# Kinetica-jl/Kinetica.jl

Measured on AMD Instinct MI355X. Metric: RHS evals/sec (batched sweep) + wall-clock per solve_network, 10k-species CRN, higher is better.
Workload: dtype f64; 1 GPU; synthetic CRN 10000 species / 50000 reactions (seed 12345), batched RHS sweep, B=4096 states per GPU with per-state Arrhenius k (500-1200 K); states_per_gpu=4096, parallelism=replicas x1 (no data-path collective)

## Files before the change

### kinetica_jl_amd/csrc/tiled_api.cpp

```cpp
#include "../../include/kinetica_hip.h"

#include <algorithm>
#include <cstdio>
#include <cmath>

#include "handle.hpp"
#include "tiled_kernels.hpp"

using namespace kin;

namespace {

int tiled_block_size(int64_t N) {
  return N <= 2300 ? 256 : (N <= 4850 ? 512 : 1024);
}

void ensure_tiled(kin_network* h) {
  if (!h->tiled_tried) {
    h->tiled_tried = true;
    h->tiled = build_tiled(h->host, tiled_block_size(h->host.N), 0);
    const TiledHost& L = h->tiled;
    if (L.ok) {
      hipStream_t s = h->stream;
      std::vector<int32_t> rxn_of_slot((size_t)L.k_len(), -1);
      for (int32_t r = 0; r < L.R; r++) if (L.slot_of_reaction[r] >= 0) rxn_of_slot[L.slot_of_reaction[r]] = r;
      h->t_rec.upload(L.rec, s);
      h->t_copy.upload(L.copy_src, s);
      h->t_kf.upload(L.kf, s); h->t_kr.upload(L.kr, s); h->t_rxn_of_slot.upload(rxn_of_slot, s); h->t_kslot.upload(L.kslot, s);
      h->t_spec_of_lib.upload(L.species_of_lib, s); h->t_lib_of_spec.upload(L.lib_of_species, s);
      if (!L.identity) { h->t_stage_lib.upload(L.stage_lib, s); h->t_stage_off.upload(L.stage_off, s); }
      KIN_HIP(hipStreamSynchronize(s));
    }
  }
  if (!h->tiled.ok) throw KinError(ERR_UNSUPPORTED, "network has no tiled layout: " + h->tiled.why);
}

void ensure_params(kin_network* h, hipStream_t) {
  if (!h->has_arrhenius) throw KinError(ERR_STATE, "Arrhenius parameters were never set");
  if (h->t_par_valid) return;
  const TiledHost& L = h->tiled;
  KIN_HIP(hipDeviceSynchronize());
  h->t_par.alloc((size_t)4 * std::max(1, L.P));
  launch_tiled_params(L.P, h->t_kf.p, h->t_kr.p, h->Ea.p, h->A.p, h->has_kmax, h->t_mult, h->t_par.p, h->stream);
  KIN_HIP(hipStreamSynchronize(h->stream));
  h->t_par_valid = true;
}

TiledView view_of(kin_network* h) {
  const TiledHost& L = h->tiled;
  TiledView v{};
  v.KL = L.KL; v.has_singles = L.has_singles ? 1 : 0;
  v.N = L.N; v.P = L.P; v.h = L.h; v.n_copy = L.n_copy; v.wbase = L.wbase; v.E = L.E; v.T = L.T;
  v.win_cnt_max = 0;
  for (int32_t c : L.win_cnt) v.win_cnt_max = std::max(v.win_cnt_max, c);
  v.rec = (const uint2*)h->t_rec.p;
  for (int32_t t = 0; t < L.T; t++) {
    v.seginfo[t] = make_int4(L.seginfo[4 * t], L.seginfo[4 * t + 1], L.seginfo[4 * t + 2], L.seginfo[4 * t + 3]);
    v.segk[t] = L.seg_k[2 * t];
    v.win_off[t] = L.win_off[t]; v.win_cnt[t] = L.win_cnt[t];
  }
  v.copy_src = h->t_copy.p;
  v.par = (const double4*)h->t_par.p;
  v.has_kmax = h->has_kmax ? 1 : 0;
  v.inv_kmax = h->has_kmax ? 1.0 / h->k_max : 0.0;
  return v;
}

void require(bool c, int code, const char* msg) {
  if (!c) throw KinError(code, msg);
}

void states_convert(kin_network* h, int64_t B, bool to_lib, const double* d_in, double* d_out, hipStream_t s) {
  const int64_t N = h->host.N;
  if (h->tiled.identity) KIN_HIP(hipMemcpyAsync(d_out, d_in, (size_t)B * N * sizeof(double), hipMemcpyDeviceToDevice, s));
  else launch_permute_staged(N, B, to_lib, h->t_stage_lib.p, h->t_stage_off.p, d_in, d_out, s);
}

}

#define KIN_TRY(h) try { KIN_HIP(hipSetDevice((h)->device));
#define KIN_CATCH(h)                                                        \
  }                                                                         \
  catch (const KinError& e) { (h)->err = e.what(); return e.code; }         \
  catch (const std::exception& e) { (h)->err = e.what(); return KIN_ERR_DEVICE; } \
  return KIN_OK;

extern "C" {

int kin_lib_layout(kin_network* h, int index_base, int64_t* k_len, int64_t* species_of_lib, int64_t* slot_of_reaction,
                   int32_t* species_identity, int64_t* info) {
  if (!h) return KIN_ERR_INVALID_ARG;
  KIN_TRY(h)
  ensure_tiled(h);
  const TiledHost& L = h->tiled;
  if (k_len) *k_len = L.k_len();
  if (species_of_lib) for (int32_t j = 0; j < L.N; j++) species_of_lib[j] = L.species_of_lib[j] + index_base;
  if (slot_of_reaction) for (int32_t r = 0; r < L.R; r++) slot_of_reaction[r] = L.slot_of_reaction[r] + index_base;
  if (species_identity) *species_identity = L.identity ? 1 : 0;
  if (info) { info[0] = L.h; info[1] = L.T; info[2] = L.P; info[3] = L.E; info[4] = L.n_copy; info[5] = L.BS; }
  KIN_CATCH(h)
}

int kin_lib_layout_host(int64_t n_species, int64_t n_reactions, const int64_t* reac_ptr, const int64_t* reac_idx,
                        const int64_t* reac_sto, const int64_t* prod_ptr, const int64_t* prod_idx, const int64_t* prod_sto,
                        int index_base, int hubs, int64_t* info, int64_t* species_of_lib, int64_t* slot_of_reaction,
                        uint64_t* rec, int32_t* rowtab, int32_t* seg_q, int32_t* win_off, int32_t* win_cnt, int32_t* copy_src,
                        int32_t* seg_k) {
  try {
    const NetworkHost H = compile_network(n_species, n_reactions, reac_ptr, reac_idx, reac_sto, prod_ptr, prod_idx, prod_sto, index_base);
    const TiledHost L = build_tiled(H, tiled_block_size(H.N), hubs);
    if (!L.ok) {
      if (getenv("KIN_TILED_DEBUG")) fprintf(stderr, "[tiled] no layout: %s\n", L.why.c_str());
      return KIN_ERR_UNSUPPORTED;
    }
    if (info) {
      info[0] = L.h; info[1] = L.T; info[2] = L.P; info[3] = L.E; info[4] = L.n_copy; info[5] = L.BS; info[6] = L.wbase;
      info[7] = L.seg_q.back(); info[8] = L.k_len(); info[9] = L.has_singles ? 1 : 0;
    }
    if (species_of_lib) for (int32_t j = 0; j < L.N; j++) species_of_lib[j] = L.species_of_lib[j];
    if (slot_of_reaction) for (int32_t r = 0; r < L.R; r++) slot_of_reaction[r] = L.slot_of_reaction[r];
    if (rec) for (int32_t p = 0; p < L.P; p++) rec[p] = (uint64_t)L.rec[2 * p] | ((uint64_t)L.rec[2 * p + 1] << 32);
    if (rowtab) std::copy(L.rowtab.begin(), L.rowtab.end(), rowtab);
    if (seg_q) std::copy(L.seg_q.begin(), L.seg_q.end(), seg_q);
    if (win_off) std::copy(L.win_off.begin(), L.win_off.end(), win_off);
    if (win_cnt) std::copy(L.win_cnt.begin(), L.win_cnt.end(), win_cnt);
    if (copy_src) std::copy(L.copy_src.begin(), L.copy_src.end(), copy_src);
    if (seg_k) std::copy(L.seg_k.begin(), L.seg_k.end(), seg_k);
  } catch (const KinError& e) {
    return e.code;
  } catch (const std::exception&) {
    return KIN_ERR_INVALID_ARG;
  }
  return KIN_OK;
}

int kin_states_to_lib_dev(kin_network* h, int64_t B, const double* d_in, double* d_out, void* stream) {
  if (!h) return KIN_ERR_INVALID_ARG;
  KIN_TRY(h)
  require(B > 0 && d_in && d_out && d_in != d_out, ERR_INVALID_ARG, "bad arguments");
  ensure_tiled(h);
  states_convert(h, B, true, d_in, d_out, stream ? (hipStream_t)stream : h->stream);
  KIN_CATCH(h)
}

int kin_states_from_lib_dev(kin_network* h, int64_t B, const double* d_in, double* d_out, void* stream) {
  if (!h) return KIN_ERR_INVALID_ARG;
  KIN_TRY(h)
  require(B > 0 && d_in && d_out && d_in != d_out, ERR_INVALID_ARG, "bad arguments");
  ensure_tiled(h);
  states_convert(h, B, false, d_in, d_out, stream ? (hipStream_t)stream : h->stream);
  KIN_CATCH(h)
}

int kin_rates_to_lib_dev(kin_network* h, int64_t B, const double* d_k, double* d_k_lib, void* stream) {
  if (!h) return KIN_ERR_INVALID_ARG;
  KIN_TRY(h)
  require(B > 0 && d_k && d_k_lib && d_k != d_k_lib, ERR_INVALID_ARG, "bad arguments");
  ensure_tiled(h);
  hipStream_t s = stream ? (hipStream_t)stream : h->stream;
  const TiledHost& L = h->tiled;
  if (L.KL == 2 * (int64_t)L.P && h->host.R % 2 == 0 && ((((uintptr_t)d_k) | ((uintptr_t)d_k_lib)) & 15) == 0)
    launch_rates_to_lib_pairs(L.P, h->host.R, B, h->t_kf.p, h->t_kr.p, d_k, d_k_lib, s);
  else
    launch_gather_rows(L.k_len(), h->host.R, B, h->t_rxn_of_slot.p, d_k, d_k_lib, s);
  KIN_CATCH(h)
}

int kin_rate_table_lib_dev(kin_network* h, const double* T, int64_t n_stops, double* d_out) {
  if (!h) return KIN_ERR_INVALID_ARG;
  KIN_TRY(h)
  require(T != nullptr && d_out != nullptr && n_stops >= 0, ERR_INVALID_ARG, "bad arguments");
  ensure_tiled(h);
  ensure_params(h, h->stream);
  h->T_stops.upload(T, n_stops, h->stream);
  TiledPadSlots pads{};
  for (int32_t q : h->tiled.pad_slots) pads.slot[pads.n++] = q;
  launch_rate_table_lib(h->tiled.P, h->tiled.KL, n_stops, h->t_par.p, h->t_kslot.p, pads, h->has_kmax, h->k_max, h->T_stops.p, d_out, h->stream);
  KIN_HIP(hipStreamSynchronize(h->stream));
  KIN_CATCH(h)
}

int kin_rhs_tiled_dev(kin_network* h, int64_t B, const double* d_u_lib, const double* d_k_lib, const double* d_T,
                      double* d_du_lib, void* stream) {
  if (!h) return KIN_ERR_INVALID_ARG;
  KIN_TRY(h)
  require(B > 0 && d_u_lib && d_du_lib, ERR_INVALID_ARG, "bad arguments");
  require((d_k_lib != nullptr) != (d_T != nullptr), ERR_INVALID_ARG, "exactly one of d_k_lib and d_T must be given");
  require((((uintptr_t)d_k_lib) & 15) == 0, ERR_INVALID_ARG, "d_k_lib must be 16-byte aligned");
  ensure_tiled(h);
  hipStream_t s = stream ? (hipStream_t)stream : h->stream;
  if (d_T) ensure_params(h, s);
  if (h->tiled.P == 0) {
    KIN_HIP(hipMemsetAsync(d_du_lib, 0, (size_t)B * h->host.N * sizeof(double), s));
    return KIN_OK;
  }
  launch_tiled_sweep(view_of(h), h->tiled.BS, h->n_cu, B, d_u_lib, d_k_lib, d_T, d_du_lib, s);
  KIN_CATCH(h)
}

int kin_rhs_batched_T_dev(kin_network* h, int64_t B, const double* d_u, const double* d_T, double* d_du, void* stream) {
  if (!h) return KIN_ERR_INVALID_ARG;
  KIN_TRY(h)
  require(B > 0 && d_u && d_T && d_du, ERR_INVALID_ARG, "bad arguments");
  ensure_tiled(h);
  hipStream_t s = stream ? (hipStream_t)stream : h->stream;
  ensure_params(h, s);
  const int64_t N = h->host.N;
  if (h->tiled.P == 0) {
    KIN_HIP(hipMemsetAsync(d_du, 0, (size_t)B * N * sizeof(double), s));
    return KIN_OK;
  }
  if (h->tiled.identity) {
    launch_tiled_sweep(view_of(h), h->tiled.BS, h->n_cu, B, d_u, nullptr, d_T, d_du, s);
  } else {
    h->t_u.alloc((size_t)B * N); h->t_du.alloc((size_t)B * N);
    states_convert(h, B, true, d_u, h->t_u.p, s);
    launch_tiled_sweep(view_of(h), h->tiled.BS, h->n_cu, B, h->t_u.p, nullptr, d_T, h->t_du.p, s);
    states_convert(h, B, false, h->t_du.p, d_du, s);
  }
  KIN_CATCH(h)
}

int kin_rhs_batched_klib_dev(kin_network* h, int64_t B, const double* d_u, const double* d_k_lib, double* d_du, void* stream) {
  if (!h) return KIN_ERR_INVALID_ARG;
  KIN_TRY(h)
  require(B > 0 && d_u && d_k_lib && d_du, ERR_INVALID_ARG, "bad arguments");
  require((((uintptr_t)d_k_lib) & 15) == 0, ERR_INVALID_ARG, "d_k_lib must be 16-byte aligned");
  ensure_tiled(h);
  hipStream_t s = stream ? (hipStream_t)stream : h->stream;
  const int64_t N = h->host.N;
  if (h->tiled.P == 0) {
    KIN_HIP(hipMemsetAsync(d_du, 0, (size_t)B * N * sizeof(double), s));
    return KIN_OK;
  }
  if (h->tiled.identity) {
    launch_tiled_sweep(view_of(h), h->tiled.BS, h->n_cu, B, d_u, d_k_lib, nullptr, d_du, s);
  } else {
    h->t_u.alloc((size_t)B * N); h->t_du.alloc((size_t)B * N);
    states_convert(h, B, true, d_u, h->t_u.p, s);
    launch_tiled_sweep(view_of(h), h->tiled.BS, h->n_cu, B, h->t_u.p, d_k_lib, nullptr, h->t_du.p, s);
    states_convert(h, B, false, h->t_du.p, d_du, s);
  }
  KIN_CATCH(h)
}

}
```

### kinetica_jl_amd/csrc/tiled_kernels.hip

```cpp
#include "tiled_kernels.hpp"

#include "exp_tab.hpp"

#ifndef KIN_TILED_SUB
#define KIN_TILED_SUB 2
#endif

namespace kin {

namespace {

template <bool TMODE, int NB_> struct Batch;
template <int NB_> struct Batch<false, NB_> { static constexpr int NB = NB_; double2 k[NB]; uint2 w[NB]; };
template <int NB_> struct Batch<true, NB_> { static constexpr int NB = NB_; double4 p[NB]; uint2 w[NB]; };

struct Labels { uint32_t l0, l1, l2, l3; };
__device__ __forceinline__ Labels decode(uint2 w) {
  return Labels{w.x & 0x3fffu, (w.x >> 14) & 0x3fffu, (w.x >> 28) | ((w.y & 0x3ffu) << 4), (w.y >> 10) & 0x3fffu};
}

}

template <int BS, bool TMODE, int UN, bool SINGLES>
__global__ __launch_bounds__(BS) void tiled_sweep_kernel(TiledView v, int B, const double* __restrict__ u,
                                                         const double* __restrict__ k_lib, const double* __restrict__ Tb,
                                                         double* __restrict__ du) {
  extern __shared__ double lds[];
  double* du_s = lds;
  double* u_s = lds + v.E;
  const double* tab_s = lds + 2 * v.E;
  const int tid = threadIdx.x;
  const int N = v.N, h = v.h, wbase = v.wbase, T = v.T;
  const size_t KL = (size_t)v.KL;

  for (int i = tid; i < v.E; i += BS) du_s[i] = 0.0;
  if (tid < TILED_DUMMY) u_s[h + tid] = 1.0;
  if (TMODE) for (int i = tid; i < TILED_EXP_TAB; i += BS) lds[2 * v.E + i] = kExp2Tab[i * (512 / TILED_EXP_TAB)];
  const int csrc = tid < v.n_copy ? v.copy_src[min(tid, max(v.n_copy - 1, 0))] : -1;
  const uint64_t dl = (uint64_t)(h + (tid & 63));
  const uint64_t ew = dl | (dl << 14) | (dl << 28) | (dl << 42) | (4ull << 56);
  const uint2 EMPTY = {(uint32_t)ew, (uint32_t)(ew >> 32)};

  const int Bm1 = B - 1;
  double un[UN];
  auto load_hubs = [&](int bb) {
    const double* ub = u + (size_t)min(bb, Bm1) * N;
#pragma unroll
    for (int x = 0; x < UN; x++) un[x] = ub[min(tid + x * BS, h - 1)];
  };
  auto store_hubs = [&]() {
#pragma unroll
    for (int x = 0; x < UN; x++) {
      const int e = tid + x * BS;
      if (e < h) u_s[e] = un[x];
    }
  };
  auto load_window = [&](int bb, int s) {
    const double* ub = u + (size_t)bb * N + v.win_off[s];
    const int cm1 = v.win_cnt[s] - 1;
#pragma unroll
    for (int x = 0; x < UN; x++) un[x] = ub[min(tid + x * BS, cm1)];
  };
  auto store_window = [&](int s) {
    const int c = v.win_cnt[s];
#pragma unroll
    for (int x = 0; x < UN; x++) {
      const int e = tid + x * BS;
      if (e < c) u_s[wbase + e] = un[x];
    }
  };

  constexpr int NB = (TMODE || UN > 5) ? 2 : 4;
  using BatchT = Batch<TMODE, NB>;
  static_assert(TILED_MIN_ROWS >= 2 * NB && (UN > 5 ? 2 : 4) % NB == 0, "segments are padded to whole batches, two at least");
  int pb = blockIdx.x, ps = 0, pi = 0;
  int4 pa = v.seginfo[0], pn = v.seginfo[T > 1 ? 1 : 0];
  int pak = SINGLES ? v.segk[0] : 0, pnk = SINGLES ? v.segk[T > 1 ? 1 : 0] : 0;
  asm volatile("" : "+s"(pa.x), "+s"(pa.y), "+s"(pa.z), "+s"(pn.x), "+s"(pn.y), "+s"(pn.z));
  if constexpr (SINGLES) asm volatile("" : "+s"(pa.w), "+s"(pn.w), "+s"(pak), "+s"(pnk));
  auto load_batch = [&](BatchT& G) {
    if (pi >= pa.z) {
      pi = 0; pa = pn; pak = pnk;
      if (++ps == T) { ps = 0; pb += gridDim.x; }
    }
    const bool live = pb < B;
    const double* kb = TMODE ? nullptr : k_lib + (size_t)min(pb, Bm1) * KL;
#pragma unroll
    for (int x = 0; x < NB; x++) {
      const int off = (pi + x) * BS + tid;
      const bool ok = live && off < pa.y;
      const int p = ok ? pa.x + off : 0;
      const uint2 w = v.rec[p];
      G.w[x].x = ok ? w.x : EMPTY.x;
      G.w[x].y = ok ? w.y : EMPTY.y;
      if constexpr (TMODE) G.p[x] = v.par[p];
      else if constexpr (!SINGLES) G.k[x] = *reinterpret_cast<const double2*>(kb + 2 * (size_t)p);
      else {
        const bool one = (off & ~63) >= pa.w;
        const size_t e = !ok ? 0 : (one ? (size_t)(pak + pa.w) + (size_t)(off & ~1) : (size_t)pak + 2 * (size_t)off);
        const double2 kk = *reinterpret_cast<const double2*>(kb + e);
        const bool odd = one && (off & 1);
        const int lo = odd ? __double2loint(kk.y) : __double2loint(kk.x), hi = odd ? __double2hiint(kk.y) : __double2hiint(kk.x);
        const int rlo = one ? 0 : __double2loint(kk.y), rhi = one ? 0 : __double2hiint(kk.y);
        G.k[x].x = __hiloint2double(hi, lo);
        G.k[x].y = __hiloint2double(rhi, rlo);
      }
    }
    pi += NB;
  };

  double RT = 1.0, inv_RT = 1.0;
#if defined(KIN_TILED_PROBE)
  double probe_acc = 0.0;
#endif
  auto consume = [&](const BatchT& G) {
    constexpr int SUB = KIN_TILED_SUB < NB ? KIN_TILED_SUB : NB;
#pragma unroll
    for (int x0 = 0; x0 < NB; x0 += SUB) {
      uint32_t fl[SUB];
      double net[SUB];
#pragma unroll
      for (int y = 0; y < SUB; y++) {
        const int x = x0 + y;
        fl[y] = __builtin_amdgcn_readfirstlane(G.w[x].y >> 24);
        const Labels L = decode(G.w[x]);
#if defined(KIN_TILED_SKIPREAD)
        double u1v = 1.0, u3v = 1.0;
        const double u0v = u_s[L.l0];
        if (fl[y] & 1u) u1v = u_s[L.l1];
        const double u2v = u_s[L.l2];
        if (fl[y] & 2u) u3v = u_s[L.l3];
        const double uf = u0v * u1v, ur = u2v * u3v;
#elif defined(KIN_TILED_PROBE) && (KIN_TILED_PROBE == 1 || KIN_TILED_PROBE == 3)
        const double uf = 1.0 + (double)L.l0, ur = 1.0 + (double)L.l2;
#else
        const double uf = u_s[L.l0] * u_s[L.l1];
        const double ur = u_s[L.l2] * u_s[L.l3];
#endif
        double kf, kr;
        if constexpr (TMODE) {
          kf = arrhenius_fast_t<TILED_EXP_TAB>(G.p[x].x, G.p[x].y, G.p[x].y, RT, inv_RT, v.has_kmax, v.inv_kmax, tab_s);
          kr = arrhenius_fast_t<TILED_EXP_TAB>(G.p[x].z, G.p[x].w, G.p[x].w, RT, inv_RT, v.has_kmax, v.inv_kmax, tab_s);
        } else {
          kf = G.k[x].x; kr = G.k[x].y;
        }
        net[y] = kf * uf - kr * ur;
      }
#pragma unroll
      for (int y = 0; y < SUB; y++) {
        if (fl[y] & 4u) continue;
        const Labels L = decode(G.w[x0 + y]);
#if defined(KIN_TILED_PROBE)
        probe_acc += net[y];
        continue;
#endif
        __hip_atomic_fetch_add(du_s + L.l0, -net[y], __ATOMIC_RELAXED, __HIP_MEMORY_SCOPE_WORKGROUP);
        if (fl[y] & 1u) __hip_atomic_fetch_add(du_s + L.l1, -net[y], __ATOMIC_RELAXED, __HIP_MEMORY_SCOPE_WORKGROUP);
        __hip_atomic_fetch_add(du_s + L.l2, net[y], __ATOMIC_RELAXED, __HIP_MEMORY_SCOPE_WORKGROUP);
        if (fl[y] & 2u) __hip_atomic_fetch_add(du_s + L.l3, net[y], __ATOMIC_RELAXED, __HIP_MEMORY_SCOPE_WORKGROUP);
      }
    }
  };

  int b = blockIdx.x;
  load_hubs(b);
  const int csrc_c = max(csrc, 0);
  double ucn = u[(size_t)min(b, Bm1) * N + csrc_c];
  double Tn = TMODE ? Tb[min(b, Bm1)] : 1.0;
  BatchT G0, G1;
  load_batch(G0);
  load_batch(G1);

  for (; b < B; b += gridDim.x) {
    double* dub = du + (size_t)b * N;
    const int bn = b + gridDim.x;
    if (TMODE) { RT = 8.314462618 * Tn; inv_RT = arrhenius_inv_RT(RT); }
#if defined(KIN_TILED_PROBE) && KIN_TILED_PROBE == 3
    for (int s = 0; s < T; s++) {
      pn = v.seginfo[ps + 1 == T ? 0 : ps + 1];
      if constexpr (SINGLES) pnk = v.segk[ps + 1 == T ? 0 : ps + 1];
      int rows = v.seginfo[s].z;
      asm volatile("" : "+s"(pn.x), "+s"(pn.y), "+s"(pn.z), "+s"(rows));
      int q = 0;
      for (; q + 2 * NB <= rows; q += 2 * NB) { consume(G0); load_batch(G0); consume(G1); load_batch(G1); }
      if (q < rows) {
        consume(G0);
#pragma unroll
        for (int x = 0; x < NB; x++) {
          G0.w[x].x = G1.w[x].x; G0.w[x].y = G1.w[x].y;
          if constexpr (TMODE) { G0.p[x].x = G1.p[x].x; G0.p[x].y = G1.p[x].y; G0.p[x].z = G1.p[x].z; G0.p[x].w = G1.p[x].w; }
          else { G0.k[x].x = G1.k[x].x; G0.k[x].y = G1.k[x].y; }
        }
        load_batch(G1);
      }
    }
    if (b >= 0) continue;
#endif
    store_hubs();
    if (csrc >= 0) u_s[h + TILED_DUMMY + tid] = ucn;
    if (v.win_cnt_max > 0) { load_window(b, 0); store_window(0); }
    __syncthreads();
    ucn = u[(size_t)min(bn, Bm1) * N + csrc_c];
    if (TMODE) Tn = Tb[min(bn, Bm1)];
    for (int s = 0; s < T; s++) {
      const bool last = s == T - 1;
      if (last) load_hubs(bn); else load_window(b, s + 1);
      pn = v.seginfo[ps + 1 == T ? 0 : ps + 1];
      if constexpr (SINGLES) pnk = v.segk[ps + 1 == T ? 0 : ps + 1];
      int rows = v.seginfo[s].z;
      asm volatile("" : "+s"(pn.x), "+s"(pn.y), "+s"(pn.z), "+s"(rows));
      if constexpr (SINGLES) asm volatile("" : "+s"(pn.w), "+s"(pnk));
      int q = 0;
      for (; q + 2 * NB <= rows; q += 2 * NB) {
        consume(G0);
        load_batch(G0);
        consume(G1);
        load_batch(G1);
      }
      if (q < rows) {
        consume(G0);
#pragma unroll
        for (int x = 0; x < NB; x++) {
          G0.w[x].x = G1.w[x].x; G0.w[x].y = G1.w[x].y;
          if constexpr (TMODE) { G0.p[x].x = G1.p[x].x; G0.p[x].y = G1.p[x].y; G0.p[x].z = G1.p[x].z; G0.p[x].w = G1.p[x].w; }
          else { G0.k[x].x = G1.k[x].x; G0.k[x].y = G1.k[x].y; }
        }
        load_batch(G1);
      }
      __syncthreads();
      if (last && v.n_copy > 0) {
        if (csrc >= 0) {
          const double a = du_s[h + TILED_DUMMY + tid];
          du_s[h + TILED_DUMMY + tid] = 0.0;
          __hip_atomic_fetch_add(du_s + csrc, a, __ATOMIC_RELAXED, __HIP_MEMORY_SCOPE_WORKGROUP);
        }
        __syncthreads();
      }
      {
        const int c = v.win_cnt[s], o = v.win_off[s];
        for (int i = tid; i < c; i += BS) { dub[o + i] = du_s[wbase + i]; du_s[wbase + i] = 0.0; }
        if (last) for (int i = tid; i < h; i += BS) { dub[i] = du_s[i]; du_s[i] = 0.0; }
      }
      if (!last) {
        store_window(s + 1);
        __syncthreads();
      }
    }
  }
#if defined(KIN_TILED_PROBE)
  if (probe_acc == 12345.678) du[0] = probe_acc;
#endif
}

__global__ __launch_bounds__(256) void gather_rows_kernel(int64_t n_dst, int64_t n_src, int B, const int32_t* __restrict__ map,
                                                          const double* __restrict__ src, double* __restrict__ dst) {
  const int64_t j = (int64_t)blockIdx.x * 256 + threadIdx.x;
  if (j >= n_dst) return;
  const int32_t m = map[j];
  for (int b = blockIdx.y; b < B; b += gridDim.y) dst[(size_t)b * n_dst + j] = m >= 0 ? src[(size_t)b * n_src + m] : 0.0;
}

template <bool TO_LIB, bool VEC2>
__global__ __launch_bounds__(256) void permute_staged_kernel(int N, const int32_t* __restrict__ stage_lib, const int32_t* __restrict__ stage_off,
                                                             const double* __restrict__ src, double* __restrict__ dst) {
  __shared__ double2 buf2[TILED_PIECE / 2];
  double* buf = (double*)buf2;
  constexpr int PT = TILED_PIECE / 256;
  const int p0 = blockIdx.x * TILED_PIECE;
  const int cnt = min(N - p0, TILED_PIECE);
  const double* s = src + (size_t)blockIdx.y * N;
  double* d = dst + (size_t)blockIdx.y * N;
  int32_t jl[PT], of[PT];
#pragma unroll
  for (int x = 0; x < PT; x++) {
    const int q = threadIdx.x + 256 * x;
    const bool ok = q < cnt;
    jl[x] = ok ? stage_lib[p0 + q] : -1;
    of[x] = ok ? stage_off[p0 + q] : 0;
  }
  if (TO_LIB) {
    if (VEC2) {
      double2 v2[PT / 2];
#pragma unroll
      for (int x = 0; x < PT / 2; x++) { const int q = threadIdx.x + 256 * x; v2[x] = 2 * q < cnt ? ((const double2*)(s + p0))[q] : make_double2(0.0, 0.0); }
#pragma unroll
      for (int x = 0; x < PT / 2; x++) { const int q = threadIdx.x + 256 * x; if (2 * q < cnt) buf2[q] = v2[x]; }
    } else {
      double v[PT];
#pragma unroll
      for (int x = 0; x < PT; x++) { const int q = threadIdx.x + 256 * x; v[x] = q < cnt ? s[p0 + q] : 0.0; }
#pragma unroll
      for (int x = 0; x < PT; x++) { const int q = threadIdx.x + 256 * x; if (q < cnt) buf[q] = v[x]; }
    }
    __syncthreads();
#pragma unroll
    for (int x = 0; x < PT; x++) if (jl[x] >= 0) d[jl[x]] = buf[of[x]];
  } else {
    double v[PT];
#pragma unroll
    for (int x = 0; x < PT; x++) v[x] = jl[x] >= 0 ? s[jl[x]] : 0.0;
#pragma unroll
    for (int x = 0; x < PT; x++) if (jl[x] >= 0) buf[of[x]] = v[x];
    __syncthreads();
    if (VEC2) {
#pragma unroll
      for (int x = 0; x < PT / 2; x++) { const int q = threadIdx.x + 256 * x; if (2 * q < cnt) ((double2*)(d + p0))[q] = buf2[q]; }
    } else {
#pragma unroll
      for (int x = 0; x < PT; x++) { const int q = threadIdx.x + 256 * x; if (q < cnt) d[p0 + q] = buf[q]; }
    }
  }
}

__global__ __launch_bounds__(256) void rates_to_lib_pairs_kernel(int P, int64_t R, int B, const int32_t* __restrict__ kf,
                                                                 const int32_t* __restrict__ kr, const double* __restrict__ src,
                                                                 double* __restrict__ dst) {
  const int p = blockIdx.x * 256 + threadIdx.x;
  if (p >= P) return;
  const int f = kf[p], r = kr[p];
  const bool straight = r == f + 1 && (f & 1) == 0, flipped = f == r + 1 && (r & 1) == 0;
  const size_t lo = (size_t)(straight ? f : (flipped ? r : 0));
  for (int b = blockIdx.y; b < B; b += gridDim.y) {
    const double* sb = src + (size_t)b * R;
    double2 v;
    if (straight || flipped) {
      const double2 w = *reinterpret_cast<const double2*>(sb + lo);
      v.x = flipped ? w.y : w.x;
      v.y = flipped ? w.x : w.y;
    } else {
      v.x = sb[f];
      v.y = r >= 0 ? sb[r] : 0.0;
    }
    *reinterpret_cast<double2*>(dst + ((size_t)b * P + p) * 2) = v;
  }
}

__global__ __launch_bounds__(256) void tiled_params_kernel(int P, const int32_t* __restrict__ kf, const int32_t* __restrict__ kr,
                                                           const double* __restrict__ Ea, const double* __restrict__ A, int has_kmax,
                                                           double t_mult, double4* __restrict__ par) {
  const int p = blockIdx.x * 256 + threadIdx.x;
  if (p >= P) return;
  const int f = kf[p], r = kr[p];
  const double cf = A[f] * 6.02214076e23 * t_mult;
  const double none = has_kmax ? __builtin_inf() : 0.0;
  double4 o;
  o.x = Ea[f]; o.y = has_kmax ? 1.0 / cf : cf;
  o.z = r >= 0 ? Ea[r] : 0.0;
  o.w = r >= 0 ? (has_kmax ? 1.0 / (A[r] * 6.02214076e23 * t_mult) : A[r] * 6.02214076e23 * t_mult) : none;
  par[p] = o;
}

__global__ __launch_bounds__(256) void rate_table_lib_kernel(int P, int64_t KL, int n_stops, const double4* __restrict__ par,
                                                             const int32_t* __restrict__ kslot, TiledPadSlots pads, int has_kmax, double inv_kmax,
                                                             const double* __restrict__ T, double* __restrict__ table) {
  constexpr int ROWS = 32;
  __shared__ double rt_s[ROWS], irt_s[ROWS];
  __shared__ double tab_s[512];
  tab_s[threadIdx.x] = kExp2Tab[threadIdx.x];
  tab_s[threadIdx.x + 256] = kExp2Tab[threadIdx.x + 256];
  const int s0 = blockIdx.y * ROWS, s1 = min(n_stops, s0 + ROWS);
  if ((int)threadIdx.x < s1 - s0) {
    const double RT = 8.314462618 * T[s0 + threadIdx.x];
    rt_s[threadIdx.x] = RT;
    irt_s[threadIdx.x] = arrhenius_inv_RT(RT);
  }
  __syncthreads();
  const int p = blockIdx.x * 256 + threadIdx.x;
  if (p < pads.n) for (int s = s0; s < s1; s++) table[(size_t)s * KL + pads.slot[p]] = 0.0;
  if (p >= P) return;
  const double4 q = par[p];
  const int32_t ks = kslot[p];
  const bool two = ks >= 0;
  const size_t slot = (size_t)(two ? ks : ~ks);
  for (int s = s0; s < s1; s++) {
    const double RT = rt_s[s - s0], inv_RT = irt_s[s - s0];
    const double kf = arrhenius_fast(q.x, q.y, q.y, RT, inv_RT, has_kmax, inv_kmax, tab_s);
    if (two) {
      const double kr = arrhenius_fast(q.z, q.w, q.w, RT, inv_RT, has_kmax, inv_kmax, tab_s);
      *reinterpret_cast<double2*>(table + (size_t)s * KL + slot) = make_double2(kf, kr);
    } else {
      table[(size_t)s * KL + slot] = kf;
    }
  }
}

void launch_gather_rows(int64_t n_dst, int64_t n_src, int64_t B, const int32_t* map, const double* src, double* dst, hipStream_t s) {
  if (n_dst == 0 || B == 0) return;
  dim3 grid((unsigned)ceil_div(n_dst, 256), (unsigned)std::min<int64_t>(B, 1024));
  hipLaunchKernelGGL(gather_rows_kernel, grid, dim3(256), 0, s, n_dst, n_src, (int)B, map, src, dst);
  KIN_HIP(hipGetLastError());
}

void launch_permute_staged(int64_t N, int64_t B, bool to_lib, const int32_t* stage_lib, const int32_t* stage_off, const double* src,
                           double* dst, hipStream_t s) {
  if (N == 0 || B == 0) return;
  for (int64_t b0 = 0; b0 < B; b0 += 65535) {
    const int64_t nb = std::min<int64_t>(65535, B - b0);
    dim3 grid((unsigned)ceil_div(N, (int64_t)TILED_PIECE), (unsigned)nb);
    const double* sp = src + (size_t)b0 * N;
    double* dp = dst + (size_t)b0 * N;
    const bool vec2 = N % 2 == 0 && ((((uintptr_t)sp) | ((uintptr_t)dp)) & 15) == 0;
    if (to_lib && vec2) hipLaunchKernelGGL((permute_staged_kernel<true, true>), grid, dim3(256), 0, s, (int)N, stage_lib, stage_off, sp, dp);
    else if (to_lib) hipLaunchKernelGGL((permute_staged_kernel<true, false>), grid, dim3(256), 0, s, (int)N, stage_lib, stage_off, sp, dp);
    else if (vec2) hipLaunchKernelGGL((permute_staged_kernel<false, true>), grid, dim3(256), 0, s, (int)N, stage_lib, stage_off, sp, dp);
    else hipLaunchKernelGGL((permute_staged_kernel<false, false>), grid, dim3(256), 0, s, (int)N, stage_lib, stage_off, sp, dp);
  }
  KIN_HIP(hipGetLastError());
}

void launch_rates_to_lib_pairs(int P, int64_t R, int64_t B, const int32_t* kf, const int32_t* kr, const double* src, double* dst,
                               hipStream_t s) {
  if (P == 0 || B == 0) return;
  dim3 grid((unsigned)ceil_div(P, 256), (unsigned)std::min<int64_t>(B, 1024));
  hipLaunchKernelGGL(rates_to_lib_pairs_kernel, grid, dim3(256), 0, s, P, R, (int)B, kf, kr, src, dst);
  KIN_HIP(hipGetLastError());
}

void launch_tiled_params(int P, const int32_t* kf, const int32_t* kr, const double* Ea, const double* A, int has_kmax,
                         double t_mult, void* par, hipStream_t s) {
  if (P == 0) return;
  hipLaunchKernelGGL(tiled_params_kernel, dim3((unsigned)ceil_div(P, 256)), dim3(256), 0, s, P, kf, kr, Ea, A, has_kmax, t_mult,
                     (double4*)par);
  KIN_HIP(hipGetLastError());
}

void launch_rate_table_lib(int P, int64_t KL, int64_t n_stops, const void* par, const int32_t* kslot, const TiledPadSlots& pads,
                           int has_kmax, double k_max, const double* T, double* table, hipStream_t s) {
  if (P == 0 || n_stops == 0) return;
  dim3 grid((unsigned)ceil_div(P, 256), (unsigned)ceil_div(n_stops, 32));
  hipLaunchKernelGGL(rate_table_lib_kernel, grid, dim3(256), 0, s, P, KL, (int)n_stops, (const double4*)par, kslot, pads, has_kmax, 1.0 / k_max, T, table);
  KIN_HIP(hipGetLastError());
}

template <int BS, bool TMODE, int UN, bool SINGLES>
static void launch_tiled_t(const TiledView& v, int grid, size_t smem, int B, const double* u, const double* k_lib, const double* Tb,
                           double* du, hipStream_t s) {
  KIN_HIP(hipFuncSetAttribute((const void*)tiled_sweep_kernel<BS, TMODE, UN, SINGLES>, hipFuncAttributeMaxDynamicSharedMemorySize, 160 * 1024));
  hipLaunchKernelGGL((tiled_sweep_kernel<BS, TMODE, UN, SINGLES>), dim3(grid), dim3(BS), smem, s, v, B, u, k_lib, Tb, du);
}

void launch_tiled_sweep(const TiledView& v, int bs, int n_cu, int64_t B, const double* u, const double* k_lib, const double* Tb,
                        double* du, hipStream_t s) {
  if (B == 0) return;
  const bool tmode = k_lib == nullptr;
  const size_t smem = ((size_t)2 * v.E + (tmode ? TILED_EXP_TAB : 0)) * 8;
  const int per_cu = (int)std::max<size_t>(1, std::min<size_t>(2048 / bs, (160 * 1024) / smem));
  const int grid = (int)std::min<int64_t>(B, (int64_t)n_cu * per_cu);
  const bool un5 = std::max(v.h, v.win_cnt_max) <= 5 * bs;
  const bool singles = !tmode && v.has_singles;
#define KIN_TILED_GO(BSZ)                                                                                  \
  do {                                                                                                     \
    if (tmode) { if (un5) launch_tiled_t<BSZ, true, 5, false>(v, grid, smem, (int)B, u, k_lib, Tb, du, s);           \
                 else launch_tiled_t<BSZ, true, 10, false>(v, grid, smem, (int)B, u, k_lib, Tb, du, s); }            \
    else if (singles) { if (un5) launch_tiled_t<BSZ, false, 5, true>(v, grid, smem, (int)B, u, k_lib, Tb, du, s);    \
                        else launch_tiled_t<BSZ, false, 10, true>(v, grid, smem, (int)B, u, k_lib, Tb, du, s); }     \
    else { if (un5) launch_tiled_t<BSZ, false, 5, false>(v, grid, smem, (int)B, u, k_lib, Tb, du, s);                \
           else launch_tiled_t<BSZ, false, 10, false>(v, grid, smem, (int)B, u, k_lib, Tb, du, s); }                 \
  } while (0)
  if (bs == 256) KIN_TILED_GO(256);
  else if (bs == 512) KIN_TILED_GO(512);
  else KIN_TILED_GO(1024);
#undef KIN_TILED_GO
  KIN_HIP(hipGetLastError());
}

}
```

Measured before the change: 10.26 million RHS evals/s.

## Streamline tiled sweep loads with padded records, 32-bit offsets and nontemporal access

Adds padding records at the end of the record array and flag bits for single-rate rows on the host, so the kernel loads a dummy record instead of selecting an empty one per lane. The singles decode moves from load time into consume. Loads and stores use 32-bit byte offsets, and the rate-constant loads and du stores become nontemporal. The odd-tail batch shuffle is replaced by a do-while loop that conditionally consumes the second batch, with segment rows rounded up to whole double batches. It also adds scheduling barriers and asm register pins to reduce VALU and address overhead, and a guard throws when offsets would not fit in 32 bits.

```diff
diff --git a/kinetica_jl_amd/csrc/tiled_api.cpp b/kinetica_jl_amd/csrc/tiled_api.cpp
--- a/kinetica_jl_amd/csrc/tiled_api.cpp
+++ b/kinetica_jl_amd/csrc/tiled_api.cpp
@@ -24,7 +24,17 @@
       hipStream_t s = h->stream;
       std::vector<int32_t> rxn_of_slot((size_t)L.k_len(), -1);
       for (int32_t r = 0; r < L.R; r++) if (L.slot_of_reaction[r] >= 0) rxn_of_slot[L.slot_of_reaction[r]] = r;
-      h->t_rec.upload(L.rec, s);
+      std::vector<uint32_t> rec = L.rec;
+      for (int32_t t = 0; t < L.T; t++) {
+        const int32_t first = L.seginfo[4 * t], cnt = L.seginfo[4 * t + 1], n2 = L.seginfo[4 * t + 3];
+        for (int32_t i = n2; i < cnt; i++) rec[2 * (size_t)(first + i) + 1] |= (1u << 27) | ((uint32_t)(i & 1) << 28);
+      }
+      for (int lane = 0; lane < TILED_DUMMY; lane++) {
+        const uint64_t dl = (uint64_t)(L.h + lane);
+        const uint64_t ew = dl | (dl << 14) | (dl << 28) | (dl << 42) | (4ull << 56);
+        rec.push_back((uint32_t)ew); rec.push_back((uint32_t)(ew >> 32));
+      }
+      h->t_rec.upload(rec, s);
       h->t_copy.upload(L.copy_src, s);
       h->t_kf.upload(L.kf, s); h->t_kr.upload(L.kr, s); h->t_rxn_of_slot.upload(rxn_of_slot, s); h->t_kslot.upload(L.kslot, s);
       h->t_spec_of_lib.upload(L.species_of_lib, s); h->t_lib_of_spec.upload(L.lib_of_species, s);
diff --git a/kinetica_jl_amd/csrc/tiled_kernels.hip b/kinetica_jl_amd/csrc/tiled_kernels.hip
--- a/kinetica_jl_amd/csrc/tiled_kernels.hip
+++ b/kinetica_jl_amd/csrc/tiled_kernels.hip
@@ -19,6 +19,30 @@
   return Labels{w.x & 0x3fffu, (w.x >> 14) & 0x3fffu, (w.x >> 28) | ((w.y & 0x3ffu) << 4), (w.y >> 10) & 0x3fffu};
 }
 
+}
+
+#ifndef KIN_TILED_NT
+#define KIN_TILED_NT 1
+#endif
+typedef double tiled_d2 __attribute__((ext_vector_type(2)));
+__device__ __forceinline__ tiled_d2 load_k2(const double* __restrict__ kb, uint32_t slot) {
+  const tiled_d2* p = reinterpret_cast<const tiled_d2*>(reinterpret_cast<const char*>(kb) + slot * 8u);
+#if KIN_TILED_NT
+  return __builtin_nontemporal_load(p);
+#else
+  return *p;
+#endif
+}
+__device__ __forceinline__ void store_du(double* __restrict__ row, uint32_t i, double x) {
+  double* p = reinterpret_cast<double*>(reinterpret_cast<char*>(row) + i * 8u);
+#if KIN_TILED_NT
+  __builtin_nontemporal_store(x, p);
+#else
+  *p = x;
+#endif
+}
+__device__ __forceinline__ double load_u(const double* __restrict__ row, uint32_t i) {
+  return *reinterpret_cast<const double*>(reinterpret_cast<const char*>(row) + i * 8u);
 }
 
 template <int BS, bool TMODE, int UN, bool SINGLES>
@@ -31,80 +55,76 @@
   const double* tab_s = lds + 2 * v.E;
   const int tid = threadIdx.x;
   const int N = v.N, h = v.h, wbase = v.wbase, T = v.T;
+  __builtin_assume(T >= 1);
   const size_t KL = (size_t)v.KL;
 
   for (int i = tid; i < v.E; i += BS) du_s[i] = 0.0;
   if (tid < TILED_DUMMY) u_s[h + tid] = 1.0;
   if (TMODE) for (int i = tid; i < TILED_EXP_TAB; i += BS) lds[2 * v.E + i] = kExp2Tab[i * (512 / TILED_EXP_TAB)];
   const int csrc = tid < v.n_copy ? v.copy_src[min(tid, max(v.n_copy - 1, 0))] : -1;
-  const uint64_t dl = (uint64_t)(h + (tid & 63));
-  const uint64_t ew = dl | (dl << 14) | (dl << 28) | (dl << 42) | (4ull << 56);
-  const uint2 EMPTY = {(uint32_t)ew, (uint32_t)(ew >> 32)};
 
   const int Bm1 = B - 1;
+  int tl = tid;
   double un[UN];
   auto load_hubs = [&](int bb) {
     const double* ub = u + (size_t)min(bb, Bm1) * N;
 #pragma unroll
-    for (int x = 0; x < UN; x++) un[x] = ub[min(tid + x * BS, h - 1)];
-  };
+    for (int x = 0; x < UN; x++) un[x] = load_u(ub, (uint32_t)min(tl + x * BS, h - 1));
+  };
+  auto stage = [&](bool in, int entry, double x) { u_s[in ? entry : h + (tl & (TILED_DUMMY - 1))] = in ? x : 1.0; };
   auto store_hubs = [&]() {
 #pragma unroll
-    for (int x = 0; x < UN; x++) {
-      const int e = tid + x * BS;
-      if (e < h) u_s[e] = un[x];
-    }
+    for (int x = 0; x < UN; x++) stage(tl + x * BS < h, tl + x * BS, un[x]);
   };
   auto load_window = [&](int bb, int s) {
     const double* ub = u + (size_t)bb * N + v.win_off[s];
     const int cm1 = v.win_cnt[s] - 1;
 #pragma unroll
-    for (int x = 0; x < UN; x++) un[x] = ub[min(tid + x * BS, cm1)];
+    for (int x = 0; x < UN; x++) un[x] = load_u(ub, (uint32_t)min(tl + x * BS, cm1));
   };
   auto store_window = [&](int s) {
     const int c = v.win_cnt[s];
 #pragma unroll
-    for (int x = 0; x < UN; x++) {
-      const int e = tid + x * BS;
-      if (e < c) u_s[wbase + e] = un[x];
-    }
+    for (int x = 0; x < UN; x++) stage(tl + x * BS < c, wbase + tl + x * BS, un[x]);
   };
 
   constexpr int NB = (TMODE || UN > 5) ? 2 : 4;
   using BatchT = Batch<TMODE, NB>;
-  static_assert(TILED_MIN_ROWS >= 2 * NB && (UN > 5 ? 2 : 4) % NB == 0, "segments are padded to whole batches, two at least");
+  static_assert(TILED_MIN_ROWS >= 2 * NB, "a segment has two batches at least");
+  auto qrows = [](int z) { return (z + 2 * NB - 1) & ~(2 * NB - 1); };
   int pb = blockIdx.x, ps = 0, pi = 0;
   int4 pa = v.seginfo[0], pn = v.seginfo[T > 1 ? 1 : 0];
   int pak = SINGLES ? v.segk[0] : 0, pnk = SINGLES ? v.segk[T > 1 ? 1 : 0] : 0;
   asm volatile("" : "+s"(pa.x), "+s"(pa.y), "+s"(pa.z), "+s"(pn.x), "+s"(pn.y), "+s"(pn.z));
   if constexpr (SINGLES) asm volatile("" : "+s"(pa.w), "+s"(pn.w), "+s"(pak), "+s"(pnk));
   auto load_batch = [&](BatchT& G) {
-    if (pi >= pa.z) {
+    if (pi >= qrows(pa.z)) {
       pi = 0; pa = pn; pak = pnk;
       if (++ps == T) { ps = 0; pb += gridDim.x; }
     }
     const bool live = pb < B;
     const double* kb = TMODE ? nullptr : k_lib + (size_t)min(pb, Bm1) * KL;
+    const uint32_t pad_rec = (uint32_t)v.P + (uint32_t)(tl & (TILED_DUMMY - 1));
 #pragma unroll
     for (int x = 0; x < NB; x++) {
-      const int off = (pi + x) * BS + tid;
+      const int off = (pi + x) * BS + tl;
       const bool ok = live && off < pa.y;
-      const int p = ok ? pa.x + off : 0;
-      const uint2 w = v.rec[p];
-      G.w[x].x = ok ? w.x : EMPTY.x;
-      G.w[x].y = ok ? w.y : EMPTY.y;
-      if constexpr (TMODE) G.p[x] = v.par[p];
-      else if constexpr (!SINGLES) G.k[x] = *reinterpret_cast<const double2*>(kb + 2 * (size_t)p);
-      else {
-        const bool one = (off & ~63) >= pa.w;
-        const size_t e = !ok ? 0 : (one ? (size_t)(pak + pa.w) + (size_t)(off & ~1) : (size_t)pak + 2 * (size_t)off);
-        const double2 kk = *reinterpret_cast<const double2*>(kb + e);
-        const bool odd = one && (off & 1);
-        const int lo = odd ? __double2loint(kk.y) : __double2loint(kk.x), hi = odd ? __double2hiint(kk.y) : __double2hiint(kk.x);
-        const int rlo = one ? 0 : __double2loint(kk.y), rhi = one ? 0 : __double2hiint(kk.y);
-        G.k[x].x = __hiloint2double(hi, lo);
-        G.k[x].y = __hiloint2double(rhi, rlo);
+      const uint2 w = *reinterpret_cast<const uint2*>(reinterpret_cast<const char*>(v.rec) + (ok ? (uint32_t)(pa.x + off) : pad_rec) * 8u);
+      G.w[x].x = w.x; G.w[x].y = w.y;
+      if constexpr (TMODE) {
+        const double4 q = v.par[ok ? pa.x + off : 0];
+        G.p[x].x = q.x; G.p[x].y = q.y; G.p[x].z = q.z; G.p[x].w = q.w;
+      } else {
+        uint32_t e;
+        if constexpr (!SINGLES) e = ok ? 2u * (uint32_t)(pa.x + off) : 0u;
+        else {
+          const bool one = (off & ~63) >= pa.w;
+          e = !ok ? 0u : (one ? (uint32_t)(pak + pa.w) + (uint32_t)(off & ~1) : (uint32_t)pak + 2u * (uint32_t)off);
+        }
+        const tiled_d2 kk = load_k2(kb, e);
+        G.k[x].x = kk.x; G.k[x].y = kk.y;
       }
+      __builtin_amdgcn_sched_barrier(0);
     }
     pi += NB;
   };
@@ -141,6 +161,12 @@
         if constexpr (TMODE) {
           kf = arrhenius_fast_t<TILED_EXP_TAB>(G.p[x].x, G.p[x].y, G.p[x].y, RT, inv_RT, v.has_kmax, v.inv_kmax, tab_s);
           kr = arrhenius_fast_t<TILED_EXP_TAB>(G.p[x].z, G.p[x].w, G.p[x].w, RT, inv_RT, v.has_kmax, v.inv_kmax, tab_s);
+        } else if constexpr (SINGLES) {
+          const bool one = fl[y] & 8u, odd = G.w[x].y & (1u << 28);
+          const int lo = odd ? __double2loint(G.k[x].y) : __double2loint(G.k[x].x), hi = odd ? __double2hiint(G.k[x].y) : __double2hiint(G.k[x].x);
+          const int rlo = one ? 0 : __double2loint(G.k[x].y), rhi = one ? 0 : __double2hiint(G.k[x].y);
+          kf = __hiloint2double(hi, lo);
+          kr = __hiloint2double(rhi, rlo);
         } else {
           kf = G.k[x].x; kr = G.k[x].y;
         }
@@ -161,11 +187,13 @@
       }
     }
   };
+  auto write_out = [&](double* __restrict__ row, double* __restrict__ src, int c) {
+    for (int i = tl; i < c; i += BS) { store_du(row, (uint32_t)i, src[i]); src[i] = 0.0; }
+  };
 
   int b = blockIdx.x;
   load_hubs(b);
-  const int csrc_c = max(csrc, 0);
-  double ucn = u[(size_t)min(b, Bm1) * N + csrc_c];
+  double ucn = u[(size_t)min(b, Bm1) * N + max(csrc, 0)];
   double Tn = TMODE ? Tb[min(b, Bm1)] : 1.0;
   BatchT G0, G1;
   load_batch(G0);
@@ -174,6 +202,7 @@
   for (; b < B; b += gridDim.x) {
     double* dub = du + (size_t)b * N;
     const int bn = b + gridDim.x;
+    asm volatile("" : "+v"(tl));
     if (TMODE) { RT = 8.314462618 * Tn; inv_RT = arrhenius_inv_RT(RT); }
 #if defined(KIN_TILED_PROBE) && KIN_TILED_PROBE == 3
     for (int s = 0; s < T; s++) {
@@ -181,29 +210,19 @@
       if constexpr (SINGLES) pnk = v.segk[ps + 1 == T ? 0 : ps + 1];
       int rows = v.seginfo[s].z;
       asm volatile("" : "+s"(pn.x), "+s"(pn.y), "+s"(pn.z), "+s"(rows));
-      int q = 0;
-      for (; q + 2 * NB <= rows; q += 2 * NB) { consume(G0); load_batch(G0); consume(G1); load_batch(G1); }
-      if (q < rows) {
-        consume(G0);
-#pragma unroll
-        for (int x = 0; x < NB; x++) {
-          G0.w[x].x = G1.w[x].x; G0.w[x].y = G1.w[x].y;
-          if constexpr (TMODE) { G0.p[x].x = G1.p[x].x; G0.p[x].y = G1.p[x].y; G0.p[x].z = G1.p[x].z; G0.p[x].w = G1.p[x].w; }
-          else { G0.k[x].x = G1.k[x].x; G0.k[x].y = G1.k[x].y; }
-        }
-        load_batch(G1);
-      }
+      for (int q = 0; q < rows; q += 2 * NB) { consume(G0); load_batch(G0); consume(G1); load_batch(G1); }
     }
     if (b >= 0) continue;
 #endif
     store_hubs();
-    if (csrc >= 0) u_s[h + TILED_DUMMY + tid] = ucn;
+    stage(csrc >= 0, h + TILED_DUMMY + tl, ucn);
     if (v.win_cnt_max > 0) { load_window(b, 0); store_window(0); }
     __syncthreads();
-    ucn = u[(size_t)min(bn, Bm1) * N + csrc_c];
+    ucn = u[(size_t)min(bn, Bm1) * N + max(csrc, 0)];
     if (TMODE) Tn = Tb[min(bn, Bm1)];
     for (int s = 0; s < T; s++) {
       const bool last = s == T - 1;
+      asm volatile("" : "+v"(tl));
       if (last) load_hubs(bn); else load_window(b, s + 1);
       pn = v.seginfo[ps + 1 == T ? 0 : ps + 1];
       if constexpr (SINGLES) pnk = v.segk[ps + 1 == T ? 0 : ps + 1];
@@ -211,36 +230,25 @@
       asm volatile("" : "+s"(pn.x), "+s"(pn.y), "+s"(pn.z), "+s"(rows));
       if constexpr (SINGLES) asm volatile("" : "+s"(pn.w), "+s"(pnk));
       int q = 0;
-      for (; q + 2 * NB <= rows; q += 2 * NB) {
+      do {
         consume(G0);
         load_batch(G0);
-        consume(G1);
+        if (q + NB < rows) consume(G1);
         load_batch(G1);
-      }
-      if (q < rows) {
-        consume(G0);
-#pragma unroll
-        for (int x = 0; x < NB; x++) {
-          G0.w[x].x = G1.w[x].x; G0.w[x].y = G1.w[x].y;
-          if constexpr (TMODE) { G0.p[x].x = G1.p[x].x; G0.p[x].y = G1.p[x].y; G0.p[x].z = G1.p[x].z; G0.p[x].w = G1.p[x].w; }
-          else { G0.k[x].x = G1.k[x].x; G0.k[x].y = G1.k[x].y; }
-        }
-        load_batch(G1);
-      }
+        q += 2 * NB;
+      } while (q < rows);
       __syncthreads();
       if (last && v.n_copy > 0) {
         if (csrc >= 0) {
-          const double a = du_s[h + TILED_DUMMY + tid];
-          du_s[h + TILED_DUMMY + tid] = 0.0;
+          const double a = du_s[h + TILED_DUMMY + tl];
+          du_s[h + TILED_DUMMY + tl] = 0.0;
           __hip_atomic_fetch_add(du_s + csrc, a, __ATOMIC_RELAXED, __HIP_MEMORY_SCOPE_WORKGROUP);
         }
         __syncthreads();
       }
-      {
-        const int c = v.win_cnt[s], o = v.win_off[s];
-        for (int i = tid; i < c; i += BS) { dub[o + i] = du_s[wbase + i]; du_s[wbase + i] = 0.0; }
-        if (last) for (int i = tid; i < h; i += BS) { dub[i] = du_s[i]; du_s[i] = 0.0; }
-      }
+      asm volatile("" : "+v"(tl));
+      write_out(dub + v.win_off[s], du_s + wbase, v.win_cnt[s]);
+      if (last) write_out(dub, du_s, h);
       if (!last) {
         store_window(s + 1);
         __syncthreads();
@@ -442,6 +450,8 @@
 void launch_tiled_sweep(const TiledView& v, int bs, int n_cu, int64_t B, const double* u, const double* k_lib, const double* Tb,
                         double* du, hipStream_t s) {
   if (B == 0) return;
+  if ((v.KL + 2) * 8 >= ((int64_t)1 << 32) || ((int64_t)v.P + TILED_DUMMY) * 8 >= ((int64_t)1 << 32))
+    throw KinError(ERR_UNSUPPORTED, "tiled sweep: a row of rate constants or the record array exceeds 4 GB");
   const bool tmode = k_lib == nullptr;
   const size_t smem = ((size_t)2 * v.E + (tmode ? TILED_EXP_TAB : 0)) * 8;
   const int per_cu = (int)std::max<size_t>(1, std::min<size_t>(2048 / bs, (160 * 1024) / smem));
```

Result: no change. 10.28 million RHS evals/s (median of 6 runs) (+0.2%).
